# jhamrick/bayesian-quadrature

Measured on AMD Instinct MI355X. Metric: bq_fit_posterior_throughput, higher is better.
Workload: dtype f64; 1 GPU; C2: d=1 N=1024 M=256 Gaussian integrand, w=dx, s=1e-3; curve_workload=C5 shard: 64 x (d=1 N=2048 M=256), w=dx, s=1e-2, on_curve=True, bordered_system=1344

## Files before the change

bayesian-quadrature_amd/csrc/k_panel.hip:

```cpp
#include "host.h"
#include "gram.h"
#include "trsm.h"
#include "slab.h"

namespace bqh {

template <int D>
void launch_assemble_d(bq_ctx *c, const double *pts, long pstride, const double *y, long ystride,
                       const GaussParams *gp, int gpstride, double *A, long lda, long astride,
                       Layout L, int batch, const FirstStep &fs, int jcols)
{
    dim3 grid((L.ntot + 127) / 128, ((jcols > 0 ? jcols : L.ntot) + 63) / 64, batch);
    if (!fs.S0) {
        hipLaunchKernelGGL(assemble_kernel<D>, grid, dim3(256), 0, c->cur, pts, pstride, y, ystride,
                           gp, gpstride, A, lda, astride, L);
        return;
    }
    const bool regs = c->cfg.first_regs != 0;
    if (regs && grid.y < 3)
        grid.y = 3;
    const long wgs = (long)grid.x * grid.y * grid.z;
    const bool w8 = c->cfg.potf2_8w && wgs <= 2L * c->cus;
#define BQ_ASM_FIRST(NW_, REGS_, STAMP_)                                                           \
    hipLaunchKernelGGL((assemble_first_kernel<D, NW_, REGS_, STAMP_>), grid, dim3(64 * NW_), 0,    \
                       c->cur, pts, pstride, y, ystride, gp, gpstride, A, lda, astride, L, fs.S0,  \
                       fs.lds, fs.sstride, fs.dinv, (long)BQ_DINV_STRIDE, fs.info, fs.scal,        \
                       fs.stamps)
    if constexpr (D == 1) {
        if (fs.stamps) {
            if (w8 && regs)
                BQ_ASM_FIRST(8, true, true);
            else if (w8)
                BQ_ASM_FIRST(8, false, true);
            else if (regs)
                BQ_ASM_FIRST(4, true, true);
            else
                BQ_ASM_FIRST(4, false, true);
            return;
        }
    }
    if (w8 && regs)
        BQ_ASM_FIRST(8, true, false);
    else if (w8)
        BQ_ASM_FIRST(8, false, false);
    else if (regs)
        BQ_ASM_FIRST(4, true, false);
    else
        BQ_ASM_FIRST(4, false, false);
#undef BQ_ASM_FIRST
}

int launch_assemble(bq_ctx *c, int d, const double *pts, long pstride, const double *y,
                    long ystride, const GaussParams *gp, int gpstride, double *A, long lda,
                    long astride, Layout L, int batch, const FirstStep &fs, int jcols)
{
    if (jcols < 0 || (jcols & 63) || jcols > L.ntot || (jcols > 0 && fs.S0))
        return fail(c, BQ_ERR_BAD_ARG, "assemble: column limit");
    if (fs.stamps && (!fs.S0 || d != 1))
        return fail(c, BQ_ERR_BAD_ARG, "assemble: the stamped first launch is one-dimensional");
    const double cols = jcols > 0 ? jcols : L.ntot;
    Bracket br(c, BQ_K_GRAM, 8.0 * cols * (L.ntot - 0.5 * cols + 0.5) * batch);
    switch (d) {
    case 1: launch_assemble_d<1>(c, pts, pstride, y, ystride, gp, gpstride, A, lda, astride, L, batch, fs, jcols); break;
    case 2: launch_assemble_d<2>(c, pts, pstride, y, ystride, gp, gpstride, A, lda, astride, L, batch, fs, jcols); break;
    case 3: launch_assemble_d<3>(c, pts, pstride, y, ystride, gp, gpstride, A, lda, astride, L, batch, fs, jcols); break;
    case 4: launch_assemble_d<4>(c, pts, pstride, y, ystride, gp, gpstride, A, lda, astride, L, batch, fs, jcols); break;
    case 5: launch_assemble_d<5>(c, pts, pstride, y, ystride, gp, gpstride, A, lda, astride, L, batch, fs, jcols); break;
    case 6: launch_assemble_d<6>(c, pts, pstride, y, ystride, gp, gpstride, A, lda, astride, L, batch, fs, jcols); break;
    case 7: launch_assemble_d<7>(c, pts, pstride, y, ystride, gp, gpstride, A, lda, astride, L, batch, fs, jcols); break;
    case 8: launch_assemble_d<8>(c, pts, pstride, y, ystride, gp, gpstride, A, lda, astride, L, batch, fs, jcols); break;
    default: return fail(c, BQ_ERR_BAD_ARG, "d must be in 1..%d", BQ_MAXD);
    }
    HIPCHK(c, hipGetLastError());
    return BQ_OK;
}

int launch_assemble_region(bq_ctx *c, const GramSeed &sd, double *A, long lda, long astride, int m,
                           int n, int batch)
{
    if (m <= 0 || n <= 0)
        return BQ_OK;
    if ((m & 63) || (n & 63) || (sd.r & 63) || (sd.c & 63))
        return fail(c, BQ_ERR_BAD_ARG, "assemble_region: multiples of 64");
    Bracket br(c, BQ_K_GRAM, 8.0 * m * n * batch);
    const dim3 grid((m + 127) / 128, n / 64, batch);
#define BQ_ASM_REGION(D_)                                                                          \
    case D_:                                                                                       \
        hipLaunchKernelGGL(assemble_region_kernel<D_>, grid, dim3(256), 0, c->cur, sd.pts,         \
                           sd.pstride, sd.y, sd.ystride, sd.gp, sd.gpstride, A, lda, astride, sd.L, \
                           sd.r, sd.c, m, n);                                                      \
        break;
    switch (sd.d) {
        BQ_ASM_REGION(1)
        BQ_ASM_REGION(2)
        BQ_ASM_REGION(3)
        BQ_ASM_REGION(4)
        BQ_ASM_REGION(5)
        BQ_ASM_REGION(6)
        BQ_ASM_REGION(7)
        BQ_ASM_REGION(8)
    default:
        return fail(c, BQ_ERR_BAD_ARG, "d must be in 1..%d", BQ_MAXD);
    }
#undef BQ_ASM_REGION
    HIPCHK(c, hipGetLastError());
    return BQ_OK;
}

int launch_potf2(bq_ctx *c, double *A, long lda, long astride, int j0, double *dinv, long dstride,
                 int *info, int batch)
{
    Bracket br(c, BQ_K_POTF2, 64.0 * 64 * 64 / 3.0 * batch);
    if (c->cfg.potf2_8w && batch <= c->cus)
        hipLaunchKernelGGL(potf2_kernel<8>, dim3(1, 1, batch), dim3(512), 0, c->cur, A, lda, astride,
                           j0, dinv, dstride, info);
    else
        hipLaunchKernelGGL(potf2_kernel<4>, dim3(1, 1, batch), dim3(256), 0, c->cur, A, lda, astride,
                           j0, dinv, dstride, info);
    HIPCHK(c, hipGetLastError());
    return BQ_OK;
}

int launch_potrf_wg(bq_ctx *c, double *A, long lda, long astride, int kb, double *rec, long rstride,
                    int *info, int col0, int batch)
{
    Bracket br(c, BQ_K_POTF2, (double)kb * kb * kb / 3.0 * batch);
    hipLaunchKernelGGL(potrf_wg_kernel, dim3(batch), dim3(512), 0, c->cur, A, lda, astride, kb, rec,
                       rstride, info, col0);
    HIPCHK(c, hipGetLastError());
    return BQ_OK;
}

int launch_trsm_blk(bq_ctx *c, double *X, long ldx, long xstride, int m, const double *L11,
                    long ldl, long lstride, const double *dinv, long dstride, int batch)
{
    if (m <= 0)
        return BQ_OK;
    Bracket br(c, BQ_K_TRSM, 64.0 * 64 * (double)m * batch);
    hipLaunchKernelGGL(trsm_blk_kernel, dim3((m + 63) / 64, 1, batch), dim3(256), 0, c->cur, X, ldx,
                       xstride, m, L11, ldl, lstride, dinv, dstride);
    HIPCHK(c, hipGetLastError());
    return BQ_OK;
}

int launch_diag_winv(bq_ctx *c, const double *L, long ldl, int npad, double *dw)
{
    hipLaunchKernelGGL(diag_winv_kernel, dim3(npad / 64), dim3(256), 0, c->stream, L, ldl, dw);
    HIPCHK(c, hipGetLastError());
    return BQ_OK;
}

int launch_panel_step(bq_ctx *c, double *A, long lda, long astride, int batch, int nrb,
                      double *Sin, double *Sout, long lds, long sstride, int K0, int j0,
                      double *dinv_in, double *dinv_out, int has_next, int first, double *SL,
                      int *info, double work)
{
    Bracket br(c, BQ_K_GEMM, work);
    const bool beside_bulk = c->sharing != 0 && (long)nrb * batch > 64;
    if (c->cfg.potf2_8w && !beside_bulk && (long)nrb * batch <= c->cus)
        hipLaunchKernelGGL(panel_step_kernel<8>, dim3(nrb, 1, batch), dim3(512), 0, c->cur, A, lda,
                           astride, Sin, Sout, lds, sstride, K0, j0, dinv_in, dinv_out,
                           (long)BQ_DINV_STRIDE, has_next, first, SL, info);
    else
        hipLaunchKernelGGL(panel_step_kernel<4>, dim3(nrb, 1, batch), dim3(256), 0, c->cur, A, lda,
                           astride, Sin, Sout, lds, sstride, K0, j0, dinv_in, dinv_out,
                           (long)BQ_DINV_STRIDE, has_next, first, SL, info);
    HIPCHK(c, hipGetLastError());
    return BQ_OK;
}

int launch_slab_first(bq_ctx *c, double *A, long lda, long astride, int batch, double *S, long lds,
                      long sstride, int ntot, double *dinv, int *info, int col0, long dstride)
{
    Bracket br(c, BQ_K_POTF2, 64.0 * 64 * 64 / 3.0 * batch);
    hipLaunchKernelGGL(slab_first_kernel, dim3(ntot / 64, 1, batch), dim3(256), 0, c->cur, A, lda,
                       astride, S, lds, sstride, ntot, dinv, dstride, info, col0);
    HIPCHK(c, hipGetLastError());
    return BQ_OK;
}

static long slab8_limit(const bq_ctx *c)
{
    return (long)(c->cfg.slab8_rounds > 1 ? c->cfg.slab8_rounds : 1) * c->cus;
}

int launch_slab_step(bq_ctx *c, double *A, long lda, long astride, int batch, double *Sin,
                     double *Sout, long lds, long sstride, int ntot, int j0, double *dinv_in,
                     double *dinv_out, int fnext, int last, int *info, int col0,
                     const SlabOut &out, long long *stamps, double work, long dstride)
{
    const int T = (ntot - j0 - 64) / 64;
    Bracket br(c, BQ_K_SYRK_SMALL, work);
    const long wgs = (long)T * (T + 1) / 2 * batch;
    const bool w8 = c->cfg.potf2_8w && wgs <= slab8_limit(c);
    const bool pipe = w8 && c->cfg.diag_pipe != 0;
#define BQ_SLAB_STEP(STAMP_, NW_, PIPE_)                                                           \
    hipLaunchKernelGGL((slab_step_kernel<STAMP_, NW_, PIPE_>), dim3(T * (T + 1) / 2, 1, batch),    \
                       dim3(64 * NW_), 0, c->cur, A, lda, astride, Sin, Sout, lds, sstride, ntot,  \
                       j0, dinv_in, dinv_out, dstride, fnext, last, info, col0,                    \
                       STAMP_ ? stamps : (long long *)nullptr, out)
    if (stamps && pipe)
        BQ_SLAB_STEP(true, 8, true);
    else if (stamps && w8)
        BQ_SLAB_STEP(true, 8, false);
    else if (stamps)
        BQ_SLAB_STEP(true, 4, false);
    else if (pipe)
        BQ_SLAB_STEP(false, 8, true);
    else if (w8)
        BQ_SLAB_STEP(false, 8, false);
    else
        BQ_SLAB_STEP(false, 4, false);
#undef BQ_SLAB_STEP
    HIPCHK(c, hipGetLastError());
    return BQ_OK;
}

}
```

bayesian-quadrature_amd/csrc/launch_config.h:

```cpp
#pragma once
#include <hip/hip_runtime.h>

#pragma GCC visibility push(default)
#include "../../include/bqhip.h"
#pragma GCC visibility pop

#include <cstdio>
#include <cstdlib>

#define BQ_LAUNCH_SWITCHES(X)                                                                       \
    X(lookahead, "BQ_LOOKAHEAD", 1)                                                                 \
                 \
    X(la_min, "BQ_LA_MIN", 3072)                                                                    \
                                 \
    X(diag_first, "BQ_DIAG_FIRST", 1)                                                               \
              \
    X(df_sweep, "BQ_DF_SWEEP", 1)                                                                   \
                                               \
    X(df_wg, "BQ_DF_WG", -1)                                                                        \
                                             \
    X(df_wg_rows, "BQ_DF_WG_ROWS", 1000)                                                            \
                       \
    X(df_early, "BQ_DF_EARLY", 1)                                                                   \
                                                  \
    X(trsv_flow, "BQ_TRSV_FLOW", 1)                                                                 \
                                                                                      \
    X(pair_border, "BQ_PAIR_BORDER", 1)                                                             \
            \
    X(solve_kcopy, "BQ_SOLVE_KCOPY", 1)                                                             \
                                              \
    X(gemm_lds, "BQ_GEMM_LDS", 1)                                                                   \
                             \
    X(fold_readout, "BQ_FOLD_READOUT", 1)                                                           \
                                                                           \
    X(asm_fuse, "BQ_ASM_FUSE", 1)                                                                   \
                                                                            \
    X(potf2_8w, "BQ_POTF2_8W", 1)                                                                   \
                           \
    X(first_regs, "BQ_FIRST_REGS", 1)                                                               \
                              \
    X(slab8_rounds, "BQ_SLAB8_ROUNDS", 1 << 20)                                                     \
                       \
    X(diag_pipe, "BQ_DIAG_PIPE", 1)                                                                 \
                        \
    X(gemm_ksplit, "BQ_GEMM_KSPLIT", 1)                                                             \
                  \
    X(gemm_tile, "BQ_GEMM_TILE", 0)                                                                 \
                                                                                     \
    X(use_graph, "BQ_GRAPH", 1)                                                                     \
               \
    X(nb_override, nullptr, 0)

struct LaunchConfig {
#define X(member, env, def) int member = def;
    BQ_LAUNCH_SWITCHES(X)
#undef X
    static LaunchConfig from_env()
    {
        LaunchConfig cfg;
        static const struct {
            const char *env;
            int LaunchConfig::*member;
        } switches[] = {
#define X(member, env, def) {env, &LaunchConfig::member},
            BQ_LAUNCH_SWITCHES(X)
#undef X
        };
        for (const auto &sw : switches)
            if (const char *e = sw.env ? std::getenv(sw.env) : nullptr)
                cfg.*sw.member = std::atoi(e);
        return cfg;
    }
    friend bool operator==(const LaunchConfig &a, const LaunchConfig &b)
    {
#define X(member, env, def) if (a.member != b.member) return false;
        BQ_LAUNCH_SWITCHES(X)
#undef X
        return true;
    }
    friend bool operator!=(const LaunchConfig &a, const LaunchConfig &b) { return !(a == b); }
};

struct CaptureStats {
    long captures = 0;
    long replays = 0;
    long drops = 0;
};

struct CapturedSeq {
    hipGraph_t graph = nullptr;
    hipGraphExec_t exec = nullptr;
    enum State { NotTried, Ready, Unavailable } state = NotTried;
    LaunchConfig cfg;
    CapturedSeq() = default;
    CapturedSeq(const CapturedSeq &) = delete;
    CapturedSeq &operator=(const CapturedSeq &) = delete;
    ~CapturedSeq() { drop(); }
    void drop()
    {
        if (exec)
            (void)hipGraphExecDestroy(exec);
        if (graph)
            (void)hipGraphDestroy(graph);
        exec = nullptr;
        graph = nullptr;
        state = NotTried;
    }
    template <class Ctx, class F>
    int run(Ctx *c, F &&enqueue)
    {
        if (!c->cfg.use_graph || c->prof || !c->own_stream || c->cur != c->stream)
            return enqueue();
        if (state == Ready && cfg != c->cfg) {
            drop();
            ++c->graphs.drops;
        }
        if (state == NotTried) {
            state = Unavailable;
            cfg = c->cfg;
            if (hipStreamBeginCapture(c->stream, hipStreamCaptureModeRelaxed) == hipSuccess) {
                const int st = enqueue();
                const hipError_t e = hipStreamEndCapture(c->stream, &graph);
                if (st == BQ_OK && e == hipSuccess && graph &&
                    hipGraphInstantiate(&exec, graph, nullptr, nullptr, 0) == hipSuccess) {
                    state = Ready;
                    ++c->graphs.captures;
                }
            }
            if (state != Ready) {
                exec = nullptr;
                drop();
                state = Unavailable;
                (void)hipGetLastError();
            }
        }
        if (state != Ready)
            return enqueue();
        const hipError_t e = hipGraphLaunch(exec, c->stream);
        if (e != hipSuccess) {
            std::snprintf(c->err, sizeof c->err, "hipGraphLaunch failed: %s", hipGetErrorString(e));
            return BQ_ERR_HIP;
        }
        ++c->graphs.replays;
        return BQ_OK;
    }
};
```

bayesian-quadrature_amd/csrc/slab.h:

```cpp
#pragma once
#include "common.h"
#include "potf2.h"
#include "solve16.h"


__device__ __forceinline__ constexpr int slab_diag_nb(int w) { return w < 2 ? 3 : 2; }
__device__ __forceinline__ constexpr int slab_diag_rb(int w, int s)
{
    return w == 0 ? (s > 0 ? 1 : 0) : (w == 1 ? 2 : 3);
}
__device__ __forceinline__ constexpr int slab_diag_cb(int w, int s)
{
    return w == 0 ? (s == 2 ? 1 : 0) : ((w == 3 ? 2 : 0) + (w >= 2 && s == 2 ? 1 : s));
}

struct SlabWg {
    double *A;
    const double *Sin;
    double *Sout;
    const double *din;
    double *dout;
    long lda, lds;
    int j0, r0, Rb, Cb, bx, by, wave, b, factor_next, last, col0;
    int *info;
    long long *stamps;
    const SlabOut &out;
};

__device__ __forceinline__ void slab_publish_block(double *Qs, int c, int w, int l15, int l4,
                                                   const double4_t &xc)
{
#pragma unroll
    for (int r = 0; r < 4; ++r)
        Qs[(16 * c + l4 + 4 * r) * 64 + 16 * w + l15] = xc[r];
}

__device__ __forceinline__ void slab_publish(double *Qs, int w, int l15, int l4,
                                             const double4_t (&x)[4])
{
#pragma unroll
    for (int c = 0; c < 4; ++c)
        slab_publish_block(Qs, c, w, l15, l4, x[c]);
}

__device__ __forceinline__ void slab_emit(const SlabOut &out, int b, int row, int col, double s)
{
    if (row == col && row >= out.npad && row < out.npad + out.M && out.var)
        out.var[(long)b * out.mstride + (row - out.npad)] = s;
    if (row == out.yrow) {
        if (col >= out.npad && col < out.npad + out.M && out.mean)
            out.mean[(long)b * out.mstride + (col - out.npad)] = -s;
        if (col == out.yrow) {
            const double qf = -s, ld = out.scal[4 * b + 1];
            out.scal[4 * b + 2] = qf;
            out.scal[4 * b + 0] = -0.5 * qf - 0.5 * ld - 0.5 * (double)out.n * 1.8378770664093453;
        }
    }
}

template <int NA>
__device__ __forceinline__ void slab_store_diag(const SlabWg &g, int w, const double4_t (&acc)[NA])
{
    const int l15 = mfma_l15(), l4 = mfma_l4();
    const bool emit = g.last && g.out.scal != nullptr;
#pragma unroll
    for (int sb = 0; sb < 3; ++sb)
        if (sb < slab_diag_nb(w)) {
            double *Cd = g.A + g.Rb + 16 * slab_diag_rb(w, sb) + l15 +
                         (long)(g.Cb + 16 * slab_diag_cb(w, sb) + l4) * g.lda;
#pragma unroll
            for (int r = 0; r < 4; ++r)
                Cd[(long)(4 * r) * g.lda] = -acc[sb][r];
            if (emit) {
                const SlabOut o = g.out;
#pragma unroll
                for (int r = 0; r < 4; ++r)
                    slab_emit(o, g.b, g.Rb + 16 * slab_diag_rb(w, sb) + l15,
                              g.Cb + 16 * slab_diag_cb(w, sb) + l4 + 4 * r, -acc[sb][r]);
            }
        }
}

template <int NA>
__device__ __forceinline__ void slab_pack_blocks8(double *Bs, int w,
                                                  const double4_t (&acc)[NA])
{
    const int l15 = mfma_l15(), l4 = mfma_l4();
#pragma unroll
    for (int sb = 0; sb < 3; ++sb)
        if (sb < slab_diag_nb(w)) {
            const int rb = slab_diag_rb(w, sb), cb = slab_diag_cb(w, sb);
#pragma unroll
            for (int r = 0; r < 4; ++r)
                Bs[256 * ((rb * (rb + 1)) / 2 + cb) + l15 + 16 * (l4 + 4 * r)] = -acc[sb][r];
        }
}

__device__ __forceinline__ void slab_load_blocks8(Potf2FT<8> &st, const double *Bs, int w, int lane)
{
    const int rb = lane >> 4, i = lane & 15;
#pragma unroll
    for (int q = 0; q < 2; ++q)
#pragma unroll
        for (int s = 0; s < 4; ++s) {
            const int c = 4 * (8 * q + w) + s;
            const int cb = c >> 4, rc = rb > cb ? rb : cb;
            const double v = Bs[256 * ((rc * (rc + 1)) / 2 + cb) + i + 16 * (c & 15)];
            st.a[q][s] = rb >= cb ? v : 0.0;
        }
}

__device__ __forceinline__ void slab_corner_factor8(double *Ab, long lda, int j0, double *dinv_b,
                                                    int *info_b, double *plds, long long *stamps,
                                                    double *logdet)
{
    const int lane = threadIdx.x & 63;
    const int w = __builtin_amdgcn_readfirstlane(threadIdx.x >> 6);
    if (stamps && threadIdx.x == 0)
        stamps[0] = (long long)__builtin_amdgcn_s_memtime();
    Potf2FT<8> st;
    slab_load_blocks8(st, plds + 4096, w, lane);
    potf2f_run<8>(st, Ab, lda, j0, dinv_b, info_b, plds, stamps, logdet);
}

__device__ __forceinline__ void slab_factor_next8(const SlabWg &g, double *plds, long long *stamps)
{
    slab_corner_factor8(g.A + g.r0 + (long)g.r0 * g.lda, g.lda, g.col0 + g.r0, g.dout, g.info + g.b,
                        plds, stamps, g.out.scal ? g.out.scal + 4 * g.b + 1 : nullptr);
}

#define BQ_SSTAMP(stamps_, k, dep, tid)                                                            \
    if (STAMP) {                                                                                   \
        asm volatile("" ::"v"(dep));                                                               \
        __builtin_amdgcn_sched_barrier(0);                                                         \
        if (blockIdx.x == 0 && blockIdx.z == 0 && threadIdx.x == (tid))                            \
            (stamps_)[k] = (long long)__builtin_amdgcn_s_memtime();                                \
        __builtin_amdgcn_sched_barrier(0);                                                         \
    }


template <bool STAMP>
__device__ __forceinline__ void slab_pipe_update(const SlabWg g, double *plds)
{
    double *const Qs = plds;
    const int l15 = mfma_l15(), l4 = mfma_l4();
    __builtin_assume(g.wave >= 4);
    const int wu = g.wave - 4;
    const int rb0 = slab_diag_rb(wu, 0), rb1 = slab_diag_rb(wu, 1), rb2 = slab_diag_rb(wu, 2);
    const int cb0 = slab_diag_cb(wu, 0), cb1 = slab_diag_cb(wu, 1), cb2 = slab_diag_cb(wu, 2);
    double4_t acc[3];
#pragma unroll
    for (int sb = 0; sb < 3; ++sb) {
        const double *Cin = g.A + g.Rb + 16 * slab_diag_rb(wu, sb) + l15 +
                            (long)(g.Cb + 16 * slab_diag_cb(wu, sb) + l4) * g.lda;
#pragma unroll
        for (int r = 0; r < 4; ++r)
            acc[sb][r] = Cin[(long)(4 * r) * g.lda];
    }
    __syncthreads();
    __builtin_amdgcn_sched_barrier(0);
#pragma unroll
    for (int sb = 0; sb < 3; ++sb)
#pragma unroll
        for (int r = 0; r < 4; ++r) {
            double v = -acc[sb][r];
            asm volatile("" : "+v"(v));
            acc[sb][r] = v;
        }
    __builtin_amdgcn_sched_barrier(0);
#pragma unroll
    for (int c = 0; c < 4; ++c) {
        if (c > 0)
            BQ_SSTAMP(g.stamps, 15 + c, acc[0][0], 256)
        __builtin_amdgcn_sched_barrier(0);
        __syncthreads();
        __builtin_amdgcn_sched_barrier(0);
        double qa[4][3], qb[4][3];
#pragma unroll
        for (int r = 0; r < 4; ++r) {
            const double *qrow = Qs + (16 * c + l4 + 4 * r) * 64 + l15;
            qa[r][0] = qrow[16 * cb0], qb[r][0] = qrow[16 * rb0];
            qa[r][1] = qrow[16 * cb1], qb[r][1] = qrow[16 * rb1];
            qa[r][2] = qrow[16 * cb2], qb[r][2] = qrow[16 * rb2];
        }
        __builtin_amdgcn_sched_barrier(0);
#pragma unroll
        for (int r = 0; r < 4; ++r) {
            acc[0] = __builtin_amdgcn_mfma_f64_16x16x4f64(qa[r][0], qb[r][0], acc[0], 0, 0, 0);
            acc[1] = __builtin_amdgcn_mfma_f64_16x16x4f64(qa[r][1], qb[r][1], acc[1], 0, 0, 0);
            acc[2] = __builtin_amdgcn_mfma_f64_16x16x4f64(qa[r][2], qb[r][2], acc[2], 0, 0, 0);
        }
    }
    BQ_SSTAMP(g.stamps, 4, acc[1][3] + acc[0][0], 256)
    if (blockIdx.x == 0 && g.factor_next) {
        slab_pack_blocks8(plds + 4096, wu, acc);
        __syncthreads();
        slab_factor_next8(g, plds, nullptr);
        return;
    }
    slab_store_diag(g, wu, acc);
}

template <bool STAMP, int C>
__device__ __forceinline__ void slab_pipe_block(const SlabWg &g, double *plds, const double (&tc)[4],
                                                Solve16Regs<> &f, double4_t (&x)[4])
{
    solve16_block<C>(tc, f, x);
    slab_publish_block(plds, C, g.wave, mfma_l15(), mfma_l4(), x[C]);
    if constexpr (C < 2)
        f.template load_lds_block<C + 2>(plds + 4096);
    if (C > 0)
        BQ_SSTAMP(g.stamps, 18 + C, x[C][3], 0)
    __syncthreads();
}

template <bool STAMP>
__device__ __forceinline__ void slab_pipe_solve(const SlabWg g, double *plds)
{
    const int l15 = mfma_l15(), l4 = mfma_l4();
    double tp[4][4];
    double *Fs = plds + 4096;
    {
        double f6[6], wv[4];
        solve16_stage_request(g.A + g.j0 + (long)g.j0 * g.lda, g.lda, g.din, f6, wv);
        solve16_load(g.Sin + g.Rb + 16 * g.wave + l15 + (long)l4 * g.lds, g.lds, tp);
        __builtin_amdgcn_sched_barrier(0);
        solve16_stage_store(Fs, f6, wv);
    }
    __syncthreads();
    Solve16Regs<> f;
    double4_t x[4];
    f.load_lds_block<0>(Fs);
    f.load_lds_block<1>(Fs);
    BQ_SSTAMP(g.stamps, 1, f.wf[0][3] + f.wf[1][3], 0)
    slab_pipe_block<STAMP, 0>(g, plds, tp[0], f, x);
    slab_pipe_block<STAMP, 1>(g, plds, tp[1], f, x);
    slab_pipe_block<STAMP, 2>(g, plds, tp[2], f, x);
    slab_pipe_block<STAMP, 3>(g, plds, tp[3], f, x);
    BQ_SSTAMP(g.stamps, 2, x[3][3], 0)
    if (g.by == 0)
        solve16_store(g.A + g.Rb + 16 * g.wave + l15 + (long)(g.j0 + l4) * g.lda, g.lda, x);
    if (blockIdx.x == 0 && g.factor_next) {
        __syncthreads();
        slab_factor_next8(g, plds, (STAMP && blockIdx.z == 0) ? g.stamps + 5 : nullptr);
    }
}

__device__ __forceinline__ void slab_upper_waves(const SlabWg g, double *plds)
{
    const int l15 = mfma_l15(), l4 = mfma_l4();
    if (g.bx != g.by) {
        __builtin_assume(g.wave >= 4);
        const int wq = g.wave - 4;
        double tq[4][4];
        solve16_load(g.Sin + g.Cb + 16 * wq + l15 + (long)l4 * g.lds, g.lds, tq);
        __syncthreads();
        Solve16Regs<> f;
        f.load_lds(plds + 4096);
        double4_t xq[4];
        solve16(tq, f, xq);
        slab_publish(plds, wq, l15, l4, xq);
        __syncthreads();
        return;
    }
    __syncthreads();
    __syncthreads();
    if (blockIdx.x == 0 && g.factor_next) {
        __syncthreads();
        slab_factor_next8(g, plds, nullptr);
    }
}

__device__ __forceinline__ void slab_update_diag(const double *Qs, int wave,
                                                 double4_t (&acc)[4])
{
    const int l15 = mfma_l15(), l4 = mfma_l4();
    const int rb0 = slab_diag_rb(wave, 0), rb1 = slab_diag_rb(wave, 1), rb2 = slab_diag_rb(wave, 2);
    const int cb0 = slab_diag_cb(wave, 0), cb1 = slab_diag_cb(wave, 1), cb2 = slab_diag_cb(wave, 2);
#pragma unroll
    for (int c = 0; c < 4; ++c)
#pragma unroll
        for (int r = 0; r < 4; ++r) {
            const double *qrow = Qs + (16 * c + l4 + 4 * r) * 64 + l15;
            acc[0] = __builtin_amdgcn_mfma_f64_16x16x4f64(qrow[16 * cb0], qrow[16 * rb0], acc[0], 0, 0, 0);
            acc[1] = __builtin_amdgcn_mfma_f64_16x16x4f64(qrow[16 * cb1], qrow[16 * rb1], acc[1], 0, 0, 0);
            acc[2] = __builtin_amdgcn_mfma_f64_16x16x4f64(qrow[16 * cb2], qrow[16 * rb2], acc[2], 0, 0, 0);
        }
}

__device__ __forceinline__ void slab_update_offdiag(const double *Qs,
                                                    const double4_t (&xp)[4], double4_t (&acc)[4])
{
    const int l15 = mfma_l15(), l4 = mfma_l4();
#pragma unroll
    for (int c = 0; c < 4; ++c)
#pragma unroll
        for (int r = 0; r < 4; ++r) {
            const double pf = xp[c][r];
            const double *qrow = Qs + (16 * c + l4 + 4 * r) * 64 + l15;
#pragma unroll
            for (int cb = 0; cb < 4; ++cb)
                acc[cb] = __builtin_amdgcn_mfma_f64_16x16x4f64(qrow[16 * cb], pf, acc[cb], 0, 0, 0);
        }
}

template <bool STAMP, int NW, bool PIPE>
__device__ __forceinline__ void slab_one_phase(const SlabWg g, double *plds)
{
    double *const Qs = plds;
    double *const Ts = plds;
    double *const Fs = plds + 4096;
    const int bx = g.bx, by = g.by, wave = g.wave, l15 = mfma_l15(), l4 = mfma_l4();
    Solve16Regs<> f;
    double tp[4][4], tq[4][4];
    double4_t acc[4];
    {
        double f6[6], wv[4];
        solve16_stage_request(g.A + g.j0 + (long)g.j0 * g.lda, g.lda, g.din, f6, wv);
        if (NW == 4)
            solve16_load(g.Sin + g.Cb + 16 * wave + l15 + (long)l4 * g.lds, g.lds, tq);
        solve16_load(g.Sin + g.Rb + 16 * wave + l15 + (long)l4 * g.lds, g.lds, tp);
        {
            const bool dg = bx == by;
#pragma unroll
            for (int cb = 0; cb < 4; ++cb) {
                const int sb = cb < 2 ? cb : 2;
                const int ro = dg ? 16 * slab_diag_rb(wave, sb) : 16 * wave;
                const int co = dg ? 16 * slab_diag_cb(wave, sb) : 16 * cb;
                const double *Cin = g.A + g.Rb + ro + l15 + (long)(g.Cb + co + l4) * g.lda;
#pragma unroll
                for (int r = 0; r < 4; ++r)
                    acc[cb][r] = Cin[(long)(4 * r) * g.lda];
            }
        }
        __builtin_amdgcn_sched_barrier(0);
        solve16_stage_store(Fs, f6, wv);
    }
    __syncthreads();
    f.load_lds(Fs);
    BQ_SSTAMP(g.stamps, 1, f.la[3][2][3] + f.wf[3][3], 0)
    double4_t xp[4];
    if (NW == 4 && bx != by) {
        double4_t xq[4];
        solve16(tq, f, xq);
        slab_publish(Qs, wave, l15, l4, xq);
    }
    solve16(tp, f, xp);
    if (bx == by)
        slab_publish(Qs, wave, l15, l4, xp);
    BQ_SSTAMP(g.stamps, 2, xp[3][3], 0)
    __builtin_amdgcn_sched_barrier(0);
#pragma unroll
    for (int cb = 0; cb < 4; ++cb)
        if (cb < 3 || bx != by) {
#pragma unroll
            for (int r = 0; r < 4; ++r) {
                double v = -acc[cb][r];
                asm volatile("" : "+v"(v));
                acc[cb][r] = v;
            }
        }
    __builtin_amdgcn_sched_barrier(0);
    if (by == 0)
        solve16_store(g.A + g.Rb + 16 * wave + l15 + (long)(g.j0 + l4) * g.lda, g.lda, xp);
    __syncthreads();
    BQ_SSTAMP(g.stamps, 3, acc[1][3] + acc[0][0], 0)
    if (bx == by)
        slab_update_diag(Qs, wave, acc);
    else
        slab_update_offdiag(Qs, xp, acc);
    BQ_SSTAMP(g.stamps, 4, acc[1][3] + acc[0][0], 0)
    if (!(NW == 8 && PIPE) && blockIdx.x == 0 && g.factor_next) {
        if constexpr (NW == 8) {
            slab_pack_blocks8(Fs, wave, acc);
            __syncthreads();
            slab_factor_next8(g, plds, (STAMP && blockIdx.z == 0) ? g.stamps + 5 : nullptr);
            return;
        }
        __syncthreads();
#pragma unroll
        for (int sb = 0; sb < 3; ++sb)
            if (sb < slab_diag_nb(wave)) {
#pragma unroll
                for (int r = 0; r < 4; ++r)
                    Ts[16 * slab_diag_rb(wave, sb) + l15 +
                       64 * (16 * slab_diag_cb(wave, sb) + l4 + 4 * r)] = -acc[sb][r];
            }
        __syncthreads();
        potf2_body<NW>(g.A + g.r0 + (long)g.r0 * g.lda, g.lda, g.col0 + g.r0, g.dout, g.info + g.b,
                       plds, Ts, 64, (STAMP && blockIdx.z == 0) ? g.stamps + 5 : nullptr,
                       g.out.scal ? g.out.scal + 4 * g.b + 1 : nullptr);
        return;
    }
    const bool to_s = by == 0 && bx > 0 && !g.last;
    double *Cout = to_s ? g.Sout + g.Rb + 16 * wave + l15 + (long)l4 * g.lds
                        : g.A + g.Rb + 16 * wave + l15 + (long)(g.Cb + l4) * g.lda;
    const long ldo = to_s ? g.lds : g.lda;
    if (bx == by) {
        slab_store_diag(g, wave, acc);
    } else {
#pragma unroll
        for (int cb = 0; cb < 4; ++cb)
#pragma unroll
            for (int r = 0; r < 4; ++r)
                Cout[(long)(16 * cb + 4 * r) * ldo] = -acc[cb][r];
        if (g.last && g.out.scal != nullptr) {
            const SlabOut o = g.out;
#pragma unroll
            for (int cb = 0; cb < 4; ++cb)
#pragma unroll
                for (int r = 0; r < 4; ++r)
                    slab_emit(o, g.b, g.Rb + 16 * wave + l15, g.Cb + 16 * cb + l4 + 4 * r,
                              -acc[cb][r]);
        }
    }
}

template <bool STAMP, int NW = 4, bool PIPE = false>
__global__ __launch_bounds__(64 * NW, NW == 4 ? 2 : 1) void slab_step_kernel(double *__restrict__ A, long lda,
                                                        long astride,
                                                        const double *__restrict__ Sin,
                                                        double *__restrict__ Sout, long lds,
                                                        long sstride, int ntot, int j0,
                                                        const double *__restrict__ din,
                                                        double *__restrict__ dout, long dstride,
                                                        int factor_next, int last,
                                                        int *__restrict__ info, int col0,
                                                        long long *stamps, SlabOut out)
{
    BQ_SSTAMP(stamps, 0, 0, 0)
    __shared__ __attribute__((aligned(16))) double plds[4096 + BQ_SLAB_FW];
    __builtin_amdgcn_s_setprio(3);
    const int b = blockIdx.z;
    const int wave = __builtin_amdgcn_readfirstlane(threadIdx.x >> 6);
    int bx, by;
    tri_decode(blockIdx.x, bx, by);
    const int r0 = j0 + 64;
    const SlabWg g = {A + (long)b * astride, Sin + (long)b * sstride, Sout + (long)b * sstride,
                      din + (long)b * dstride, dout + (long)b * dstride, lda, lds, j0, r0,
                      r0 + 64 * bx, r0 + 64 * by, bx, by, wave, b, factor_next, last, col0, info,
                      stamps, out};
    if constexpr (NW == 8 && PIPE) {
        if (g.bx == g.by) {
            if (g.wave >= 4) {
                slab_pipe_update<STAMP>(g, plds);
                return;
            }
            slab_pipe_solve<STAMP>(g, plds);
            return;
        }
    }
    if (NW == 8 && g.wave >= 4) {
        slab_upper_waves(g, plds);
        return;
    }
    slab_one_phase<STAMP, NW, PIPE>(g, plds);
}
#undef BQ_SSTAMP


template <int D, int NW>
__device__ __forceinline__ void first_block_regs(Potf2FT<NW> &st, const double *__restrict__ pts,
                                                 const GaussParams &gm, double *__restrict__ A,
                                                 long lda, const Layout &L, int wv, int lane)
{
    constexpr int NG = 16 / NW;
    constexpr int GQ = 4 * NG * D <= 32 ? NG : 1;
    Layout L0 = L;
    L0.yrow = -1;
    GaussParams g;
    g.c = gm.c, g.s2 = gm.s2;
#pragma unroll
    for (int k = 0; k < D; ++k)
        g.nh[k] = gm.nh[k];
    const bool pi = lane < L.n;
    double xi[D];
#pragma unroll
    for (int k = 0; k < D; ++k)
        xi[k] = pts[k + (long)(pi ? lane : 0) * D];
#pragma unroll
    for (int q0 = 0; q0 < NG; q0 += GQ) {
        double xj[GQ][4][D];
#pragma unroll
        for (int q = 0; q < GQ; ++q)
#pragma unroll
            for (int s = 0; s < 4; ++s) {
                const int c = 4 * (NW * (q0 + q) + wv) + s;
#pragma unroll
                for (int k = 0; k < D; ++k)
                    xj[q][s][k] = pts[k + (long)(c < L.n ? c : 0) * D];
            }
        __builtin_amdgcn_sched_barrier(0);
#pragma unroll
        for (int q = 0; q < GQ; ++q)
#pragma unroll
            for (int s = 0; s < 4; ++s) {
                const int c = 4 * (NW * (q0 + q) + wv) + s;
                st.a[q0 + q][s] =
                    bordered_entry_flat<D>(lane, c, pi, c < L.n, xi, xj[q][s], g, L0, 0.0);
            }
    }
#pragma unroll
    for (int q = 0; q < NG; ++q)
#pragma unroll
        for (int s = 0; s < 4; ++s)
            PIN(st.a[q][s]);
#pragma unroll
    for (int q = 0; q < NG; ++q)
#pragma unroll
        for (int s = 0; s < 4; ++s) {
            const int c = 4 * (NW * q + wv) + s;
            if (lane < c)
                A[lane + (long)c * lda] = st.a[q][s];
        }
}

template <int D, int NW = 4, bool REGS = true, bool STAMP = false>
__global__ __launch_bounds__(64 * NW) void assemble_first_kernel(
    const double *__restrict__ pts, long pstride, const double *__restrict__ y, long ystride,
    const GaussParams *__restrict__ gp, int gpstride, double *__restrict__ A, long lda,
    long astride, Layout L, double *__restrict__ S0, long lds, long sstride,
    double *__restrict__ dinv, long dstride, int *__restrict__ info, double *__restrict__ scal,
    long long *stamps)
{
    __shared__ __attribute__((aligned(16))) double plds[BQ_POTF2_LDS_DOUBLES];
    const int b = blockIdx.z;
    const bool corner = blockIdx.x == 0 && blockIdx.y == 0;
    long long *const st0 = (STAMP && corner && b == 0) ? stamps : nullptr;
    if (st0 && threadIdx.x == 0)
        st0[0] = (long long)__builtin_amdgcn_s_memtime();
    A += (long)b * astride;
    if constexpr (REGS) {
        if (blockIdx.x == 0 && blockIdx.y == 2) {
            if (NW == 4 || threadIdx.x < 256)
                assemble_tile<D>(pts + (long)b * pstride, y + (long)b * ystride,
                                 gp[(long)b * gpstride], A, lda, L, S0 + (long)b * sstride, lds, 64,
                                 0, 128);
            return;
        }
        if (corner) {
            __builtin_amdgcn_s_setprio(3);
            const int lane = threadIdx.x & 63;
            Potf2FT<NW> st;
            first_block_regs<D, NW>(st, pts + (long)b * pstride, gp[(long)b * gpstride], A, lda, L,
                                    (int)(threadIdx.x >> 6), lane);
            if (st0) {
                asm volatile("" ::"v"(st.a[0][0]));
                if (threadIdx.x == 0)
                    st0[1] = st0[2] = (long long)__builtin_amdgcn_s_memtime();
            }
            potf2f_run<NW>(st, A, lda, 0, dinv + (long)b * dstride, info + b, plds,
                           st0 ? st0 + 2 : nullptr, scal ? scal + 4 * b + 1 : nullptr, L.n, true);
            return;
        }
    }
    if (NW == 4 || threadIdx.x < 256)
        assemble_tile<D>(pts + (long)b * pstride, y + (long)b * ystride, gp[(long)b * gpstride],
                         A, lda, L, S0 + (long)b * sstride, lds);
    if (!REGS && corner) {
        if (threadIdx.x == 0) {
            info[b] = 0;
            if (scal)
                scal[4 * b + 1] = 0.0;
        }
        asm volatile("s_waitcnt vmcnt(0)" ::: "memory");
        __syncthreads();
        if (st0 && threadIdx.x == 0)
            st0[1] = (long long)__builtin_amdgcn_s_memtime();
        __builtin_amdgcn_s_setprio(3);
        potf2_body<NW>(A, lda, 0, dinv + (long)b * dstride, info + b, plds, nullptr, 0,
                       st0 ? st0 + 2 : nullptr, scal ? scal + 4 * b + 1 : nullptr, L.n);
    }
}

__global__ __launch_bounds__(256) void slab_first_kernel(double *__restrict__ A, long lda,
                                                         long astride, double *__restrict__ S,
                                                         long lds, long sstride, int ntot,
                                                         double *__restrict__ dinv, long dstride,
                                                         int *__restrict__ info, int col0)
{
    __shared__ __attribute__((aligned(16))) double plds[BQ_POTF2_LDS_DOUBLES];
    const int b = blockIdx.z;
    A += (long)b * astride;
    if (blockIdx.x == 0) {
        __builtin_amdgcn_s_setprio(3);
        potf2_body(A, lda, col0, dinv + (long)b * dstride, info + b, plds);
        return;
    }
    const int i = 64 * (int)blockIdx.x + (threadIdx.x & 63);
    const int jb = (threadIdx.x >> 6) * 16;
    if (i < ntot) {
        double *dst = S + (long)b * sstride + i + (long)jb * lds;
        const double *src = A + i + (long)jb * lda;
#pragma unroll
        for (int j = 0; j < 16; ++j)
            dst[(long)j * lds] = src[(long)j * lda];
    }
}

template <int NW = 4>
__global__ __launch_bounds__(64 * NW) void panel_step_kernel(double *__restrict__ A, long lda,
                                                         long astride,
                                                         const double *__restrict__ Sin,
                                                         double *__restrict__ Sout, long lds,
                                                         long sstride, int K0, int j0,
                                                         const double *__restrict__ din,
                                                         double *__restrict__ dout, long dstride,
                                                         int has_next, int first,
                                                         double *__restrict__ SL,
                                                         int *__restrict__ info)
{
    __shared__ __attribute__((aligned(16))) double plds[BQ_POTF2_LDS_DOUBLES];
    double *const Qs = plds;
    double *const Ts = plds;
    __builtin_amdgcn_s_setprio(3);
    const int b = blockIdx.z;
    const int lane = threadIdx.x & 63;
    const int wave = __builtin_amdgcn_readfirstlane(threadIdx.x >> 6);
    A += (long)b * astride;
    Sin += (long)b * sstride;
    Sout += (long)b * sstride;
    din += (long)b * dstride;
    dout += (long)b * dstride;
    const int r0 = j0 + 64;
    const int Rb = r0 + 64 * blockIdx.x;
    const int l15 = lane & 15, l4 = lane >> 4;
    SL += (long)b * 4096;
    const double *Sp = first ? A + (long)j0 * lda : Sin;
    const long ldsp = first ? lda : lds;
    if (!first && j0 - K0 == 64 && blockIdx.x == 0) {
        double *dst = A + j0 + (long)(j0 - 64) * lda;
        for (int e = threadIdx.x; e < 4096; e += 64 * NW)
            dst[(e & 63) + (long)(e >> 6) * lda] = SL[e];
    }
    if (NW == 8 && wave >= 4 && (!has_next || blockIdx.x == 0)) {
        if (!has_next)
            return;
        __syncthreads();
        __syncthreads();
        __syncthreads();
        potf2_body<8>(A + r0 + (long)r0 * lda, lda, r0, dout, info + b, plds, Ts, 64);
        return;
    }

    Solve16Regs<> f;
    f.load_global(A + j0 + (long)j0 * lda, lda, din, l15, l4);
    double4_t xp[4];
    if (has_next && blockIdx.x != 0 && (NW == 4 || wave >= 4)) {
        const int wq = wave & 3;
        double4_t xq[4];
        double tq[4][4];
        solve16_load(Sp + r0 + 16 * wq + l15 + (long)l4 * ldsp, ldsp, tq);
        solve16(tq, f, xq);
        slab_publish(Qs, wq, l15, l4, xq);
        if (NW == 8) {
            __syncthreads();
            return;
        }
    }
    {
        double tp[4][4];
        solve16_load(Sp + Rb + 16 * wave + l15 + (long)l4 * ldsp, ldsp, tp);
        solve16(tp, f, xp);
    }
    {
        const bool side = first && has_next && blockIdx.x == 0 && gridDim.x > 1;
        double *Lw = side ? SL + 16 * wave + l15 + 64 * l4
                          : A + Rb + 16 * wave + l15 + (long)(j0 + l4) * lda;
        solve16_store(Lw, side ? 64 : lda, xp);
    }
    if (!has_next)
        return;
    if (blockIdx.x == 0)
        slab_publish(Qs, wave, l15, l4, xp);
    const double *Cin = A + Rb + 16 * wave + l15 + (long)(r0 + l4) * lda;
    double4_t acc[4];
#pragma unroll
    for (int cb = 0; cb < 4; ++cb)
#pragma unroll
        for (int r = 0; r < 4; ++r)
            acc[cb][r] = -Cin[(long)(16 * cb + 4 * r) * lda];
    {
        const double *Pg = A + Rb + 16 * wave + l15 + (long)(K0 + l4) * lda;
        const double *Qg = A + r0 + l15 + (long)(K0 + l4) * lda;
        const int kend = j0 - K0;
        double pa[4], qa[4][4], pb[4], qb[4][4];
#define BQ_PANEL_LOAD(PF, QF, KK)                                                                  \
    _Pragma("unroll") for (int t = 0; t < 4; ++t)                                                  \
    {                                                                                              \
        PF[t] = Pg[(long)((KK) + 4 * t) * lda];                                                    \
        _Pragma("unroll") for (int cb = 0; cb < 4; ++cb) QF[t][cb] =                               \
            Qg[16 * cb + (long)((KK) + 4 * t) * lda];                                              \
    }
#define BQ_PANEL_MFMA(PF, QF)                                                                      \
    _Pragma("unroll") for (int t = 0; t < 4; ++t) _Pragma("unroll") for (int cb = 0; cb < 4; ++cb) \
        acc[cb] = __builtin_amdgcn_mfma_f64_16x16x4f64(QF[t][cb], PF[t], acc[cb], 0, 0, 0);
        if (kend > 0) {
            BQ_PANEL_LOAD(pa, qa, 0)
            for (int kk = 0; kk < kend; kk += 32) {
                BQ_PANEL_LOAD(pb, qb, kk + 16)
                __builtin_amdgcn_sched_barrier(0);
                BQ_PANEL_MFMA(pa, qa)
                __builtin_amdgcn_sched_barrier(0);
                const int kn = kk + 32 < kend ? kk + 32 : kk;
                BQ_PANEL_LOAD(pa, qa, kn)
                __builtin_amdgcn_sched_barrier(0);
                BQ_PANEL_MFMA(pb, qb)
                __builtin_amdgcn_sched_barrier(0);
            }
        }
#undef BQ_PANEL_LOAD
#undef BQ_PANEL_MFMA
    }
    __syncthreads();
#pragma unroll
    for (int c = 0; c < 4; ++c)
#pragma unroll
        for (int r = 0; r < 4; ++r) {
            const double pf = xp[c][r];
            const double *qrow = Qs + (16 * c + l4 + 4 * r) * 64 + l15;
#pragma unroll
            for (int cb = 0; cb < 4; ++cb)
                acc[cb] = __builtin_amdgcn_mfma_f64_16x16x4f64(qrow[16 * cb], pf, acc[cb], 0, 0, 0);
        }
    if (blockIdx.x == 0) {
        __syncthreads();
#pragma unroll
        for (int cb = 0; cb < 4; ++cb)
#pragma unroll
            for (int r = 0; r < 4; ++r)
                Ts[16 * wave + l15 + 64 * (16 * cb + l4 + 4 * r)] = -acc[cb][r];
        __syncthreads();
        potf2_body<NW>(A + r0 + (long)r0 * lda, lda, r0, dout, info + b, plds, Ts, 64);
        return;
    }
    double *Cout = Sout + Rb + 16 * wave + l15 + (long)l4 * lds;
#pragma unroll
    for (int cb = 0; cb < 4; ++cb)
#pragma unroll
        for (int r = 0; r < 4; ++r)
            Cout[(long)(16 * cb + 4 * r) * lds] = -acc[cb][r];
}

__device__ __forceinline__ void wg_update32(double *__restrict__ C, long ldc,
                                            const double *__restrict__ P,
                                            const double *__restrict__ Q, long ldp, int row0,
                                            int col0, int lane)
{
    const int l15 = lane & 15, l4 = lane >> 4;
    double pa[16][2], qa[16][2], cold[2][2][4];
#pragma unroll
    for (int h = 0; h < 2; ++h) {
        const double *pp = P + row0 + 16 * h + l15 + (long)l4 * ldp;
        const double *qq = Q + col0 + 16 * h + l15 + (long)l4 * ldp;
#pragma unroll
        for (int ks = 0; ks < 16; ++ks) {
            pa[ks][h] = pp[(long)(4 * ks) * ldp];
            qa[ks][h] = qq[(long)(4 * ks) * ldp];
        }
    }
#pragma unroll
    for (int tm = 0; tm < 2; ++tm)
#pragma unroll
        for (int tn = 0; tn < 2; ++tn)
#pragma unroll
            for (int rr = 0; rr < 4; ++rr)
                cold[tm][tn][rr] =
                    C[(row0 + 16 * tm + l15) + (long)(col0 + 16 * tn + l4 + 4 * rr) * ldc];
    __builtin_amdgcn_sched_barrier(0);
    double4_t acc[2][2];
#pragma unroll
    for (int tm = 0; tm < 2; ++tm)
#pragma unroll
        for (int tn = 0; tn < 2; ++tn)
            acc[tm][tn] = (double4_t){0.0, 0.0, 0.0, 0.0};
#pragma unroll
    for (int ks = 0; ks < 16; ++ks)
#pragma unroll
        for (int tm = 0; tm < 2; ++tm)
#pragma unroll
            for (int tn = 0; tn < 2; ++tn)
                acc[tm][tn] =
                    __builtin_amdgcn_mfma_f64_16x16x4f64(qa[ks][tn], pa[ks][tm], acc[tm][tn], 0, 0, 0);
#pragma unroll
    for (int tm = 0; tm < 2; ++tm)
#pragma unroll
        for (int tn = 0; tn < 2; ++tn) {
            if (col0 + 16 * tn >= row0 + 16 * tm + 16)
                continue;
#pragma unroll
            for (int rr = 0; rr < 4; ++rr)
                C[(row0 + 16 * tm + l15) + (long)(col0 + 16 * tn + l4 + 4 * rr) * ldc] =
                    cold[tm][tn][rr] - acc[tm][tn][rr];
        }
}

__global__ __launch_bounds__(512) void potrf_wg_kernel(double *__restrict__ A, long lda,
                                                       long astride, int kb,
                                                       double *__restrict__ rec, long rstride,
                                                       int *__restrict__ info, int col0)
{
    __shared__ __attribute__((aligned(16))) double plds[BQ_POTF2_LDS_DOUBLES];
    __builtin_amdgcn_s_setprio(3);
    const int b = blockIdx.x;
    A += (long)b * astride;
    rec += (long)b * rstride;
    const int lane = threadIdx.x & 63;
    const int wave = __builtin_amdgcn_readfirstlane(threadIdx.x >> 6);
    const int l15 = lane & 15, l4 = lane >> 4;
    const int ns = kb >> 6;
    for (int s = 0; s < ns; ++s) {
        double *Ass = A + 64 * s + (long)(64 * s) * lda;
        double *rs = rec + (long)s * BQ_DINV_HALF;
        potf2_body<8>(Ass, lda, col0 + 64 * s, rs, info + b, plds);
        asm volatile("s_waitcnt vmcnt(0)" ::: "memory");
        __syncthreads();
        const int nr = ns - s - 1;
        if (nr == 0)
            break;
        const int r0 = 64 * (s + 1);
        {
            Solve16Regs<> f;
            f.load_global(Ass, lda, rs, l15, l4);
            for (int task = wave; task < 4 * nr; task += 8) {
                double *Xr = A + r0 + 16 * task + l15 + (long)(64 * s + l4) * lda;
                double t[4][4];
                double4_t x[4];
                solve16_load(Xr, lda, t);
                solve16(t, f, x);
                solve16_store(Xr, lda, x);
            }
        }
        asm volatile("s_waitcnt vmcnt(0)" ::: "memory");
        __syncthreads();
        {
            const double *Pn = A + r0 + (long)(64 * s) * lda;
            double *Cn = A + r0 + (long)r0 * lda;
            const int ntask = 4 * (nr * (nr + 1) / 2);
            for (int task = wave; task < ntask; task += 8) {
                int ti, tj;
                tri_decode(task >> 2, ti, tj);
                const int q = task & 3;
                const int row0 = 64 * ti + 32 * (q & 1), cl0 = 64 * tj + 32 * (q >> 1);
                if (cl0 > row0)
                    continue;
                wg_update32(Cn, lda, Pn, Pn, lda, row0, cl0, lane);
            }
        }
        asm volatile("s_waitcnt vmcnt(0)" ::: "memory");
        __syncthreads();
    }
}
```

Baseline: 4522 problems/s.

## Specialize slab step tile stores: write-through atomics, skip stores on last emit step

Adds a TILES template parameter to the slab step kernel with three variants. On the final folded step that emits outputs, tile stores are dropped and workgroups whose tiles never feed the output row exit early. On single-round eight-wave steps that factor the next panel, workgroups with blockIdx.x > 2 use agent-scope relaxed atomic stores. The aim is to cut wasted global writes and shorten the wait before the next panel factor, at the cost of more kernel instantiations and extra timing stamp instrumentation.

```diff
diff --git a/bayesian-quadrature_amd/csrc/k_panel.hip b/bayesian-quadrature_amd/csrc/k_panel.hip
--- a/bayesian-quadrature_amd/csrc/k_panel.hip
+++ b/bayesian-quadrature_amd/csrc/k_panel.hip
@@ -194,23 +194,37 @@
     const long wgs = (long)T * (T + 1) / 2 * batch;
     const bool w8 = c->cfg.potf2_8w && wgs <= slab8_limit(c);
     const bool pipe = w8 && c->cfg.diag_pipe != 0;
-#define BQ_SLAB_STEP(STAMP_, NW_, PIPE_)                                                           \
-    hipLaunchKernelGGL((slab_step_kernel<STAMP_, NW_, PIPE_>), dim3(T * (T + 1) / 2, 1, batch),    \
-                       dim3(64 * NW_), 0, c->cur, A, lda, astride, Sin, Sout, lds, sstride, ntot,  \
-                       j0, dinv_in, dinv_out, dstride, fnext, last, info, col0,                    \
-                       STAMP_ ? stamps : (long long *)nullptr, out)
-    if (stamps && pipe)
-        BQ_SLAB_STEP(true, 8, true);
-    else if (stamps && w8)
-        BQ_SLAB_STEP(true, 8, false);
-    else if (stamps)
-        BQ_SLAB_STEP(true, 4, false);
-    else if (pipe)
-        BQ_SLAB_STEP(false, 8, true);
-    else if (w8)
-        BQ_SLAB_STEP(false, 8, false);
-    else
-        BQ_SLAB_STEP(false, 4, false);
+    const bool wt = w8 && c->cfg.tile_wt != 0 && fnext && wgs <= c->cus;
+    const bool emit = last && out.scal != nullptr;
+#define BQ_SLAB_STEP(STAMP_, NW_, PIPE_, TILES_)                                                   \
+    hipLaunchKernelGGL((slab_step_kernel<STAMP_, NW_, PIPE_, TILES_>),                             \
+                       dim3(T * (T + 1) / 2, 1, batch), dim3(64 * NW_), 0, c->cur, A, lda,         \
+                       astride, Sin, Sout, lds, sstride, ntot, j0, dinv_in, dinv_out, dstride,     \
+                       fnext, last, info, col0, STAMP_ ? stamps : (long long *)nullptr, out)
+#define BQ_SLAB_STEP_NW(STAMP_, NW_, PIPE_)                                                        \
+    do {                                                                                           \
+        if (emit)                                                                                  \
+            BQ_SLAB_STEP(STAMP_, NW_, PIPE_, SLAB_TILES_EMIT);                                     \
+        else if (NW_ == 8 && wt)                                                                   \
+            BQ_SLAB_STEP(STAMP_, 8, PIPE_, SLAB_TILES_WT);                                         \
+        else                                                                                       \
+            BQ_SLAB_STEP(STAMP_, NW_, PIPE_, SLAB_TILES_PLAIN);                                    \
+    } while (0)
+#define BQ_SLAB_STEP_ANY(STAMP_)                                                                   \
+    do {                                                                                           \
+        if (pipe)                                                                                  \
+            BQ_SLAB_STEP_NW(STAMP_, 8, true);                                                      \
+        else if (w8)                                                                               \
+            BQ_SLAB_STEP_NW(STAMP_, 8, false);                                                     \
+        else                                                                                       \
+            BQ_SLAB_STEP_NW(STAMP_, 4, false);                                                     \
+    } while (0)
+    if (stamps)
+        BQ_SLAB_STEP_ANY(true);
+    else
+        BQ_SLAB_STEP_ANY(false);
+#undef BQ_SLAB_STEP_ANY
+#undef BQ_SLAB_STEP_NW
 #undef BQ_SLAB_STEP
     HIPCHK(c, hipGetLastError());
     return BQ_OK;
diff --git a/bayesian-quadrature_amd/csrc/launch_config.h b/bayesian-quadrature_amd/csrc/launch_config.h
--- a/bayesian-quadrature_amd/csrc/launch_config.h
+++ b/bayesian-quadrature_amd/csrc/launch_config.h
@@ -42,6 +42,8 @@
     X(slab8_rounds, "BQ_SLAB8_ROUNDS", 1 << 20)                                                     \
                        \
     X(diag_pipe, "BQ_DIAG_PIPE", 1)                                                                 \
+                                                               \
+    X(tile_wt, "BQ_TILE_WT", 1)                                                                     \
                         \
     X(gemm_ksplit, "BQ_GEMM_KSPLIT", 1)                                                             \
                   \
diff --git a/bayesian-quadrature_amd/csrc/slab.h b/bayesian-quadrature_amd/csrc/slab.h
--- a/bayesian-quadrature_amd/csrc/slab.h
+++ b/bayesian-quadrature_amd/csrc/slab.h
@@ -22,6 +22,7 @@
     double *dout;
     long lda, lds;
     int j0, r0, Rb, Cb, bx, by, wave, b, factor_next, last, col0;
+    int swg;
     int *info;
     long long *stamps;
     const SlabOut &out;
@@ -58,19 +59,49 @@
     }
 }
 
-template <int NA>
+enum { SLAB_TILES_PLAIN = 0, SLAB_TILES_WT = 1, SLAB_TILES_EMIT = 2 };
+
+template <int TILES>
+__device__ __forceinline__ void slab_tile_store(double *p, double v, bool wt)
+{
+    static_assert(TILES != SLAB_TILES_EMIT, "the folded last step stores no tile");
+    if (TILES == SLAB_TILES_WT && wt)
+        __hip_atomic_store(p, v, __ATOMIC_RELAXED, __HIP_MEMORY_SCOPE_AGENT);
+    else
+        *p = v;
+}
+
+__device__ __forceinline__ bool slab_wg_wt() { return blockIdx.x > 2; }
+
+__device__ __forceinline__ bool slab_tile_dead(const SlabOut &out, int bx, int by, int Rb)
+{
+    return bx != by && by > 0 && (out.yrow < Rb || out.yrow >= Rb + 64);
+}
+
+template <int TILES>
+__device__ __forceinline__ bool slab_emits(const SlabWg &g)
+{
+    if constexpr (TILES == SLAB_TILES_PLAIN)
+        return g.last && g.out.scal != nullptr;
+    return TILES == SLAB_TILES_EMIT;
+}
+
+template <int TILES, int NA>
 __device__ __forceinline__ void slab_store_diag(const SlabWg &g, int w, const double4_t (&acc)[NA])
 {
     const int l15 = mfma_l15(), l4 = mfma_l4();
-    const bool emit = g.last && g.out.scal != nullptr;
+    const bool wt = slab_wg_wt();
+    const bool emit = slab_emits<TILES>(g);
 #pragma unroll
     for (int sb = 0; sb < 3; ++sb)
         if (sb < slab_diag_nb(w)) {
             double *Cd = g.A + g.Rb + 16 * slab_diag_rb(w, sb) + l15 +
                          (long)(g.Cb + 16 * slab_diag_cb(w, sb) + l4) * g.lda;
-#pragma unroll
-            for (int r = 0; r < 4; ++r)
-                Cd[(long)(4 * r) * g.lda] = -acc[sb][r];
+            if constexpr (TILES != SLAB_TILES_EMIT) {
+#pragma unroll
+                for (int r = 0; r < 4; ++r)
+                    slab_tile_store<TILES>(Cd + (long)(4 * r) * g.lda, -acc[sb][r], wt);
+            }
             if (emit) {
                 const SlabOut o = g.out;
 #pragma unroll
@@ -129,17 +160,27 @@
                         plds, stamps, g.out.scal ? g.out.scal + 4 * g.b + 1 : nullptr);
 }
 
-#define BQ_SSTAMP(stamps_, k, dep, tid)                                                            \
+#define BQ_SSTAMP_AT(stamps_, k, dep, wg, tid, clock)                                              \
     if (STAMP) {                                                                                   \
         asm volatile("" ::"v"(dep));                                                               \
         __builtin_amdgcn_sched_barrier(0);                                                         \
-        if (blockIdx.x == 0 && blockIdx.z == 0 && threadIdx.x == (tid))                            \
-            (stamps_)[k] = (long long)__builtin_amdgcn_s_memtime();                                \
+        if ((int)blockIdx.x == (wg) && blockIdx.z == 0 && threadIdx.x == (tid))                    \
+            (stamps_)[k] = (long long)clock();                                                     \
         __builtin_amdgcn_sched_barrier(0);                                                         \
     }
-
-
-template <bool STAMP>
+#define BQ_SSTAMP(stamps_, k, dep, tid)                                                            \
+    BQ_SSTAMP_AT(stamps_, k, dep, 0, tid, __builtin_amdgcn_s_memtime)
+#define BQ_SSTAMP_STORES(stamps_, k, dep, wg, tid, drained)                                        \
+    if (STAMP) {                                                                                   \
+        if (drained)                                                                               \
+            asm volatile("s_waitcnt vmcnt(0)" ::: "memory");                                       \
+        BQ_SSTAMP_AT(stamps_, k, dep, wg, tid, __builtin_amdgcn_s_memrealtime)                     \
+        if ((wg) != 0)                                                                             \
+            BQ_SSTAMP_AT(stamps_, (k) + 3, dep, wg, tid, __builtin_amdgcn_s_memtime)               \
+    }
+
+
+template <bool STAMP, int TILES>
 __device__ __forceinline__ void slab_pipe_update(const SlabWg g, double *plds)
 {
     double *const Qs = plds;
@@ -198,7 +239,8 @@
         slab_factor_next8(g, plds, nullptr);
         return;
     }
-    slab_store_diag(g, wu, acc);
+    slab_store_diag<TILES>(g, wu, acc);
+    BQ_SSTAMP_STORES(g.stamps, 25, 0, 0, 256, true)
 }
 
 template <bool STAMP, int C>
@@ -243,6 +285,7 @@
     if (blockIdx.x == 0 && g.factor_next) {
         __syncthreads();
         slab_factor_next8(g, plds, (STAMP && blockIdx.z == 0) ? g.stamps + 5 : nullptr);
+        BQ_SSTAMP_STORES(g.stamps, 25, 0, 0, 0, false)
     }
 }
 
@@ -304,7 +347,7 @@
         }
 }
 
-template <bool STAMP, int NW, bool PIPE>
+template <bool STAMP, int NW, bool PIPE, int TILES>
 __device__ __forceinline__ void slab_one_phase(const SlabWg g, double *plds)
 {
     double *const Qs = plds;
@@ -370,11 +413,13 @@
     else
         slab_update_offdiag(Qs, xp, acc);
     BQ_SSTAMP(g.stamps, 4, acc[1][3] + acc[0][0], 0)
+    BQ_SSTAMP_STORES(g.stamps, 27, acc[1][3] + acc[0][0], g.swg, 0, false)
     if (!(NW == 8 && PIPE) && blockIdx.x == 0 && g.factor_next) {
         if constexpr (NW == 8) {
             slab_pack_blocks8(Fs, wave, acc);
             __syncthreads();
             slab_factor_next8(g, plds, (STAMP && blockIdx.z == 0) ? g.stamps + 5 : nullptr);
+            BQ_SSTAMP_STORES(g.stamps, 25, 0, 0, 0, false)
             return;
         }
         __syncthreads();
@@ -397,14 +442,18 @@
                         : g.A + g.Rb + 16 * wave + l15 + (long)(g.Cb + l4) * g.lda;
     const long ldo = to_s ? g.lds : g.lda;
     if (bx == by) {
-        slab_store_diag(g, wave, acc);
+        slab_store_diag<TILES>(g, wave, acc);
+        BQ_SSTAMP_STORES(g.stamps, 25, 0, 0, 0, true)
     } else {
-#pragma unroll
-        for (int cb = 0; cb < 4; ++cb)
-#pragma unroll
-            for (int r = 0; r < 4; ++r)
-                Cout[(long)(16 * cb + 4 * r) * ldo] = -acc[cb][r];
-        if (g.last && g.out.scal != nullptr) {
+        if constexpr (TILES != SLAB_TILES_EMIT) {
+            const bool wt = slab_wg_wt();
+#pragma unroll
+            for (int cb = 0; cb < 4; ++cb)
+#pragma unroll
+                for (int r = 0; r < 4; ++r)
+                    slab_tile_store<TILES>(Cout + (long)(16 * cb + 4 * r) * ldo, -acc[cb][r], wt);
+        }
+        if (slab_emits<TILES>(g)) {
             const SlabOut o = g.out;
 #pragma unroll
             for (int cb = 0; cb < 4; ++cb)
@@ -413,10 +462,11 @@
                     slab_emit(o, g.b, g.Rb + 16 * wave + l15, g.Cb + 16 * cb + l4 + 4 * r,
                               -acc[cb][r]);
         }
-    }
-}
-
-template <bool STAMP, int NW = 4, bool PIPE = false>
+        BQ_SSTAMP_STORES(g.stamps, 28, 0, g.swg, 0, true)
+    }
+}
+
+template <bool STAMP, int NW = 4, bool PIPE = false, int TILES = SLAB_TILES_PLAIN>
 __global__ __launch_bounds__(64 * NW, NW == 4 ? 2 : 1) void slab_step_kernel(double *__restrict__ A, long lda,
                                                         long astride,
                                                         const double *__restrict__ Sin,
@@ -428,7 +478,9 @@
                                                         int *__restrict__ info, int col0,
                                                         long long *stamps, SlabOut out)
 {
+    static_assert(NW == 8 || TILES != SLAB_TILES_WT, "write-through: the one-round eight-wave steps");
     BQ_SSTAMP(stamps, 0, 0, 0)
+    BQ_SSTAMP_STORES(stamps, 24, 0, 0, 0, false)
     __shared__ __attribute__((aligned(16))) double plds[4096 + BQ_SLAB_FW];
     __builtin_amdgcn_s_setprio(3);
     const int b = blockIdx.z;
@@ -436,14 +488,20 @@
     int bx, by;
     tri_decode(blockIdx.x, bx, by);
     const int r0 = j0 + 64;
+    if constexpr (TILES == SLAB_TILES_EMIT) {
+        if (slab_tile_dead(out, bx, by, r0 + 64 * bx))
+            return;
+    }
+    const int swg = STAMP && gridDim.x >= 6 ? (int)gridDim.x - (ntot - r0) / 64 + 1 : -1;
+    BQ_SSTAMP_STORES(stamps, 26, 0, swg, 0, false)
     const SlabWg g = {A + (long)b * astride, Sin + (long)b * sstride, Sout + (long)b * sstride,
                       din + (long)b * dstride, dout + (long)b * dstride, lda, lds, j0, r0,
-                      r0 + 64 * bx, r0 + 64 * by, bx, by, wave, b, factor_next, last, col0, info,
-                      stamps, out};
+                      r0 + 64 * bx, r0 + 64 * by, bx, by, wave, b, factor_next, last, col0, swg,
+                      info, stamps, out};
     if constexpr (NW == 8 && PIPE) {
         if (g.bx == g.by) {
             if (g.wave >= 4) {
-                slab_pipe_update<STAMP>(g, plds);
+                slab_pipe_update<STAMP, TILES>(g, plds);
                 return;
             }
             slab_pipe_solve<STAMP>(g, plds);
@@ -454,9 +512,11 @@
         slab_upper_waves(g, plds);
         return;
     }
-    slab_one_phase<STAMP, NW, PIPE>(g, plds);
-}
+    slab_one_phase<STAMP, NW, PIPE, TILES>(g, plds);
+}
+#undef BQ_SSTAMP_STORES
 #undef BQ_SSTAMP
+#undef BQ_SSTAMP_AT
 
 
 template <int D, int NW>
```

New measurement: 4654 problems/s, median of 6. 1.03x the previous value.
